# bibendovsky/oalsfxpp

Measured on AMD Instinct MI355X. Metric: Msamples/sec EAX reverb, 256-frame buffers, batch=4096; % HBM roofline, higher is better.
Workload: dtype f32

## Files before the change

### oalsfxpp_amd/csrc/hip/wave_effects_body.hpp

```cpp
#ifndef OALSFX_HIP_WAVE_EFFECTS_BODY_HPP
#define OALSFX_HIP_WAVE_EFFECTS_BODY_HPP

#include "common.hpp"

namespace oalsfx_hip {

namespace wfx {

constexpr int kRow = 68;
constexpr int kLdsRows = 20;
constexpr int kCoefBase = kLdsRows * kRow;
constexpr int kLdsFloats = kCoefBase + 32;

typedef __attribute__((address_space(1))) float GlobalFloat;
typedef const __attribute__((address_space(4))) oalsfx_slot_params ConstSlotParams;

struct Coef { float b0, b1, b2, a1, a2; };
template <class B> __device__ __forceinline__ Coef coef(const B& b) { return Coef{b.b0, b.b1, b.b2, b.a1, b.a2}; }

__device__ __forceinline__ void wave_sync()
{
    __builtin_amdgcn_fence(__ATOMIC_RELEASE, "wavefront");
    __builtin_amdgcn_wave_barrier();
    __builtin_amdgcn_fence(__ATOMIC_ACQUIRE, "wavefront");
}

template <int N>
__device__ __forceinline__ void chain_biquad_whole(float* row, float a1, float a2)
{
    static_assert(N % 32 == 0, "two blocks of sixteen per round");
    float y1 = row[3], y2 = row[2];
    auto step4 = [&](float4& v) {
        v.x = (v.x - (a1 * y1)) - (a2 * y2);
        v.y = (v.y - (a1 * v.x)) - (a2 * y1);
        v.z = (v.z - (a1 * v.y)) - (a2 * v.x);
        v.w = (v.w - (a1 * v.z)) - (a2 * v.y);
        y2 = v.z;
        y1 = v.w;
    };
    float4* r4 = reinterpret_cast<float4*>(row + 4);
    float4 a0 = r4[0], a1v = r4[1], a2v = r4[2], a3 = r4[3];
    float4 b0 = r4[4], b1 = r4[5], b2 = r4[6], b3 = r4[7];
    step4(a0); step4(a1v); step4(a2v); step4(a3);
    r4[0] = a0; r4[1] = a1v; r4[2] = a2v; r4[3] = a3;
    a0 = r4[8]; a1v = r4[9]; a2v = r4[10]; a3 = r4[11];
    step4(b0); step4(b1); step4(b2); step4(b3);
#pragma unroll 1
    for (int q = 8; q < N / 4; q += 8) {
        r4[q - 4] = b0; r4[q - 3] = b1; r4[q - 2] = b2; r4[q - 1] = b3;
        b0 = r4[q + 4]; b1 = r4[q + 5]; b2 = r4[q + 6]; b3 = r4[q + 7];
        step4(a0); step4(a1v); step4(a2v); step4(a3);
        r4[q + 0] = a0; r4[q + 1] = a1v; r4[q + 2] = a2v; r4[q + 3] = a3;
        a0 = r4[q + 8]; a1v = r4[q + 9]; a2v = r4[q + 10]; a3 = r4[q + 11];
        step4(b0); step4(b1); step4(b2); step4(b3);
    }
    r4[N / 4 - 4] = b0; r4[N / 4 - 3] = b1; r4[N / 4 - 2] = b2; r4[N / 4 - 1] = b3;
}

__device__ __forceinline__ void chain_biquad(float* row, int lo, int hi, float a1, float a2)
{
    float y1 = row[4 + lo - 1], y2 = row[4 + lo - 2];
    int i = lo;
    auto step4 = [&](float4& v) {
        v.x = (v.x - (a1 * y1)) - (a2 * y2);
        v.y = (v.y - (a1 * v.x)) - (a2 * y1);
        v.z = (v.z - (a1 * v.y)) - (a2 * v.x);
        v.w = (v.w - (a1 * v.z)) - (a2 * v.y);
        y2 = v.z;
        y1 = v.w;
    };
    if ((lo & 3) == 0 && lo + 16 <= hi) {
        float4* r4 = reinterpret_cast<float4*>(row + 4);
        float4 c0 = r4[(lo >> 2) + 0], c1 = r4[(lo >> 2) + 1], c2 = r4[(lo >> 2) + 2], c3 = r4[(lo >> 2) + 3];
        for (; i + 32 <= hi; i += 32) {
            const int q = i >> 2;
            float4 n0 = r4[q + 4], n1 = r4[q + 5], n2 = r4[q + 6], n3 = r4[q + 7];
            step4(c0); step4(c1); step4(c2); step4(c3);
            r4[q + 0] = c0; r4[q + 1] = c1; r4[q + 2] = c2; r4[q + 3] = c3;
            if (i + 48 <= hi) { c0 = r4[q + 8]; c1 = r4[q + 9]; c2 = r4[q + 10]; c3 = r4[q + 11]; }
            step4(n0); step4(n1); step4(n2); step4(n3);
            r4[q + 4] = n0; r4[q + 5] = n1; r4[q + 6] = n2; r4[q + 7] = n3;
        }
        if (i + 16 <= hi) {
            const int q = i >> 2;
            step4(c0); step4(c1); step4(c2); step4(c3);
            r4[q + 0] = c0; r4[q + 1] = c1; r4[q + 2] = c2; r4[q + 3] = c3;
            i += 16;
        }
    }
    for (; i < hi; ++i) {
        const float y = (row[4 + i] - (a1 * y1)) - (a2 * y2);
        row[4 + i] = y;
        y2 = y1;
        y1 = y;
    }
}

__device__ __forceinline__ void chain_first_order(float* row, int n, float c)
{
    float prev = row[3];
    int i = 0;
    if (n >= 16) {
        float4* r4 = reinterpret_cast<float4*>(row + 4);
        float4 c0 = r4[0], c1 = r4[1], c2 = r4[2], c3 = r4[3];
        auto step4 = [&](float4& v) {
            v.x = v.x + (c * prev);
            v.y = v.y + (c * v.x);
            v.z = v.z + (c * v.y);
            v.w = v.w + (c * v.z);
            prev = v.w;
        };
        for (; i + 32 <= n; i += 32) {
            const int q = i >> 2;
            float4 n0 = r4[q + 4], n1 = r4[q + 5], n2 = r4[q + 6], n3 = r4[q + 7];
            step4(c0); step4(c1); step4(c2); step4(c3);
            r4[q + 0] = c0; r4[q + 1] = c1; r4[q + 2] = c2; r4[q + 3] = c3;
            if (i + 48 <= n) { c0 = r4[q + 8]; c1 = r4[q + 9]; c2 = r4[q + 10]; c3 = r4[q + 11]; }
            step4(n0); step4(n1); step4(n2); step4(n3);
            r4[q + 4] = n0; r4[q + 5] = n1; r4[q + 6] = n2; r4[q + 7] = n3;
        }
        if (i + 16 <= n) {
            const int q = i >> 2;
            step4(c0); step4(c1); step4(c2); step4(c3);
            r4[q + 0] = c0; r4[q + 1] = c1; r4[q + 2] = c2; r4[q + 3] = c3;
            i += 16;
        }
    }
    for (; i < n; ++i) {
        prev = row[4 + i] + (c * prev);
        row[4 + i] = prev;
    }
}

__device__ __forceinline__ void advance_row(float* row, int n)
{
    if (n >= 2) {
        const float a = row[4 + n - 2], b = row[4 + n - 1];
        row[2] = a; row[3] = b;
    } else if (n == 1) {
        row[2] = row[3]; row[3] = row[4];
    }
}

__device__ __forceinline__ void load_hist(float* xrow, float* yrow, const oalsfx_hist_t& h)
{
    xrow[2] = h.x[1]; xrow[3] = h.x[0];
    yrow[2] = h.y[1]; yrow[3] = h.y[0];
}

__device__ __forceinline__ void store_hist(const float* xrow, const float* yrow, oalsfx_hist_t& h)
{
    h.x[1] = xrow[2]; h.x[0] = xrow[3];
    h.y[1] = yrow[2]; h.y[0] = yrow[3];
}

template <class T, class = void> struct LagOf { static constexpr int value = 0; };
template <class T> struct LagOf<T, decltype(void(T::kLag))> { static constexpr int value = T::kLag; };

struct Inst {
    ConstSlotParams* sp;
    oalsfx_slot_state* ss;
    GlobalFloat* ring;
    float* lds;
    int lane;
    int channels;
    bool coop;
    int wib;
    int duty;
    mutable int phase;
    float* group_lds;
    int group_stride;
};

__device__ __forceinline__ void lds_barrier()
{
    asm volatile("s_waitcnt lgkmcnt(0)\n\ts_barrier" ::: "memory");
}

template <class F>
__device__ __forceinline__ void chain_phase(const Inst& I, int lines, F&& f)
{
    if (!I.coop) {
        wave_sync();
        if (I.lane < lines) f(I.lds, I.lane);
        wave_sync();
    } else {
        const int duty = (I.duty + I.phase++) & 3;
        lds_barrier();
        if (I.wib == duty && I.lane < 4 * lines) f(I.group_lds + (I.lane / lines) * I.group_stride, I.lane % lines);
        lds_barrier();
    }
}

__device__ __forceinline__ float std_max(float a, float b) { return (a < b) ? b : a; }
__device__ __forceinline__ float std_min(float a, float b) { return (b < a) ? b : a; }

template <int CH, class G>
__device__ __forceinline__ void pan(float out[CH], int channels, const G& gains, float v)
{
#pragma unroll
    for (int c = 0; c < CH; ++c) {
        const float g = gains[c];
        if (c < channels && audible(g)) out[c] += g * v;
    }
}

struct NullW {
    __device__ void init(const Inst&) {}
    template <int CH> __device__ void tile(const Inst&, const float*, float*, int) {}
    __device__ void finish(const Inst&) {}
};

struct DedicatedW {
    __device__ void init(const Inst&) {}
    template <int CH> __device__ void tile(const Inst& I, const float* wet, float* out, int)
    {
        const auto& p = I.sp->u.dedicated;
#pragma unroll
        for (int c = 0; c < CH; ++c) {
            const float g = p.gains[c];
            if (c < I.channels && audible(g)) out[c] += wet[0] * g;
        }
    }
    __device__ void finish(const Inst&) {}
};

struct ModDelayW {
    int offset;
    float v_next[2];
    bool have_next, may_ask;
    __device__ void init(const Inst& I)
    {
        const auto& p = I.sp->u.moddelay;
        offset = I.ss->u.moddelay.offset;
        may_ask = p.delay - static_cast<int>(fabsf(p.depth)) - 1 >= 128;
        have_next = false;
        v_next[0] = v_next[1] = 0.0F;
    }
    template <class P> __device__ static int lfo_delay(const P& p, int phase)
    {
        if (p.waveform == 1) return static_cast<int>((1.0F - fabsf(2.0F - (p.lfo_scale * phase))) * p.depth) + p.delay;
        return static_cast<int>(glibc_sinf(p.lfo_scale * phase) * p.depth) + p.delay;
    }
    template <int CH> __device__ void tile(const Inst& I, const float* wet, float* out, int L)
    {
        const auto& p = I.sp->u.moddelay;
        const int lane = I.lane;
        const unsigned mask = static_cast<unsigned>(p.ring_len - 1);
        const int o = offset + lane;
        const float in = wet[0];
        const float fb = p.feedback;
        float t[2];
        int d[2];
        bool inside[2];
        float v[2];
        if (have_next) {
#pragma unroll
            for (int k = 0; k < 2; ++k) {
                d[k] = 128;
                inside[k] = false;
                v[k] = lane < L ? v_next[k] : in;
            }
        } else {
#pragma unroll
            for (int k = 0; k < 2; ++k) {
                const GlobalFloat* buf = I.ring + (k ? p.ring_len : 0);
                const int phase = (k ? o + p.lfo_disp : o) % p.lfo_range;
                d[k] = lfo_delay(p, phase);
                inside[k] = d[k] > 0 && lane - d[k] >= 0;
                v[k] = in;
                if (lane < L && d[k] != 0 && !inside[k]) v[k] = buf[static_cast<unsigned>(o - d[k]) & mask];
            }
        }
        have_next = false;
        if (may_ask && L == 64) {
            int dn[2];
#pragma unroll
            for (int k = 0; k < 2; ++k) dn[k] = lfo_delay(p, (k ? o + 64 + p.lfo_disp : o + 64) % p.lfo_range);
            have_next = __ballot(dn[0] < 128 || dn[1] < 128) == 0ULL;
            if (have_next) {
#pragma unroll
                for (int k = 0; k < 2; ++k) v_next[k] = (I.ring + (k ? p.ring_len : 0))[static_cast<unsigned>(o + 64 - dn[k]) & mask];
            }
        }
        float val[2] = {0.0F, 0.0F};
        t[0] = t[1] = 0.0F;
        int s[2] = {0, 0};
#pragma unroll
        for (int k = 0; k < 2; ++k) {
            const unsigned long long in_tile = __ballot(inside[k] && lane < L);
            if (in_tile == 0ULL) continue;
            const int d0 = __builtin_amdgcn_readlane(d[k], static_cast<int>(__builtin_ctzll(in_tile)));
            if (d0 > 16 || __ballot(lane >= d0 && lane < L && d[k] != d0) != 0ULL) continue;
            const int chain = lane % d0, step = lane / d0;
            float* row = I.lds + chain * kRow;
            const float head_t = v[k] * fb;
            if (lane < L) row[3 + step] = step == 0 ? in + head_t : in;
            wave_sync();
            if (lane < d0 && lane < L) chain_first_order(I.lds + lane * kRow, (L - lane + d0 - 1) / d0 - 1, fb);
            wave_sync();
            if (lane < L) {
                val[k] = row[3 + step];
                t[k] = step == 0 ? head_t : row[2 + step] * fb;
            }
            wave_sync();
            s[k] = L;
        }
        while (s[0] < L || s[1] < L) {
            int e[2];
            float handed[2];
#pragma unroll
            for (int k = 0; k < 2; ++k) {
                const bool blocked = lane >= s[k] && lane < L && inside[k] && lane - d[k] >= s[k];
                const unsigned long long nb = __ballot(blocked);
                e[k] = nb ? static_cast<int>(__builtin_ctzll(nb)) : L;
                handed[k] = __shfl(val[k], inside[k] ? lane - d[k] : lane);
            }
#pragma unroll
            for (int k = 0; k < 2; ++k) {
                if (lane >= s[k] && lane < L && lane < e[k]) {
                    if (inside[k]) v[k] = handed[k];
                    t[k] = v[k] * fb;
                    val[k] = in + t[k];
                }
                s[k] = max(s[k], e[k]);
            }
        }
#pragma unroll
        for (int k = 0; k < 2; ++k) {
            GlobalFloat* buf = I.ring + (k ? p.ring_len : 0);
            if (lane < L) buf[static_cast<unsigned>(o) & mask] = val[k];
        }
#pragma unroll
        for (int k = 0; k < 2; ++k) pan<CH>(out, I.channels, p.gains[k], t[k]);
        offset += L;
        wave_sync();
    }
    __device__ void finish(const Inst& I)
    {
        if (I.lane == 0) I.ss->u.moddelay.offset = offset;
    }
};

struct CompressorW {
    __device__ void init(const Inst& I)
    {
        if (I.lane == 0) {
            I.lds[3] = I.ss->u.compressor.gain_control;
            I.lds[0] = I.sp->u.compressor.attack_rate;
            I.lds[1] = I.sp->u.compressor.release_rate;
        }
        wave_sync();
    }
    template <int CH> __device__ void tile(const Inst& I, const float* wet, float* out, int L)
    {
        const auto& p = I.sp->u.compressor;
        float* row = I.lds;
        float amplitude = 1.0F;
        if (p.enabled) {
            amplitude = fabsf(wet[0]);
            amplitude = std_max(amplitude + fabsf(wet[1]), std_max(amplitude + fabsf(wet[2]), amplitude + fabsf(wet[3])));
        }
        row[4 + I.lane] = amplitude;
        chain_phase(I, 1, [L](float* row, int) {
            float gc = row[3];
            const float attack = row[0], release = row[1];
            auto follow = [&](float a) {
                if (a > gc) gc = std_min(gc + attack, a);
                else if (a < gc) gc = std_max(gc - release, a);
                return gc;
            };
            int i = 0;
            if (L >= 4) {
                float4 a = *reinterpret_cast<const float4*>(row + 4);
                for (; i + 4 <= L; i += 4) {
                    float4 an = a;
                    if (i + 8 <= L) an = *reinterpret_cast<const float4*>(row + 8 + i);
                    float4 g;
                    g.x = follow(a.x); g.y = follow(a.y); g.z = follow(a.z); g.w = follow(a.w);
                    *reinterpret_cast<float4*>(row + 4 + i) = g;
                    a = an;
                }
            }
            for (; i < L; ++i) row[4 + i] = follow(row[4 + i]);
            row[3] = gc;
        });
        const float output = 1.0F / std_min(2.0F, std_max(0.5F, row[4 + I.lane]));
        wave_sync();
#pragma unroll
        for (int j = 0; j < 4; ++j) pan<CH>(out, I.channels, p.gains[j], wet[j] * output);
    }
    __device__ void finish(const Inst& I)
    {
        if (I.lane == 0) I.ss->u.compressor.gain_control = I.lds[3];
    }
};

struct EqualizerW {
    static constexpr int kBlock = 16;
    __device__ void init(const Inst& I)
    {
        const oalsfx_equalizer_state& s = I.ss->u.equalizer;
        if (I.lane < 16) {
            const int b = I.lane >> 2, ch = I.lane & 3;
            load_hist(I.lds + (b * 4 + ch) * kRow, I.lds + ((b + 1) * 4 + ch) * kRow, s.hist[b][ch]);
        }
        if (I.lane < 4) {
            const auto& band = I.sp->u.equalizer.band[I.lane];
            float* cf = I.lds + kCoefBase + 8 * I.lane;
            cf[0] = band.b0; cf[1] = band.b1; cf[2] = band.b2; cf[3] = band.a1; cf[4] = band.a2;
        }
        wave_sync();
    }
    __device__ static void filter_block(const float* xrow, float* yrow, int n0, int n1, const float* cf)
    {
        const float b0 = cf[0], b1 = cf[1], b2 = cf[2], a1 = cf[3], a2 = cf[4];
        float x1 = xrow[4 + n0 - 1], x2 = xrow[4 + n0 - 2], y1 = yrow[4 + n0 - 1], y2 = yrow[4 + n0 - 2];
        auto step = [&](float x0) {
            const float u = ((b0 * x0) + (b1 * x1)) + (b2 * x2);
            const float y = (u - (a1 * y1)) - (a2 * y2);
            x2 = x1; x1 = x0; y2 = y1; y1 = y;
            return y;
        };
        if (n1 - n0 == kBlock) {
            const float4* x4 = reinterpret_cast<const float4*>(xrow + 4 + n0);
            float4* y4 = reinterpret_cast<float4*>(yrow + 4 + n0);
            float4 v[4] = {x4[0], x4[1], x4[2], x4[3]};
#pragma unroll
            for (int k = 0; k < 4; ++k) {
                v[k].x = step(v[k].x); v[k].y = step(v[k].y); v[k].z = step(v[k].z); v[k].w = step(v[k].w);
            }
#pragma unroll
            for (int k = 0; k < 4; ++k) y4[k] = v[k];
        } else {
            for (int n = n0; n < n1; ++n) yrow[4 + n] = step(xrow[4 + n]);
        }
    }
    template <int CH> __device__ void tile(const Inst& I, const float* wet, float* out, int L)
    {
        const auto& p = I.sp->u.equalizer;
        const int lane = I.lane;
#pragma unroll
        for (int ch = 0; ch < 4; ++ch) I.lds[ch * kRow + 4 + lane] = wet[ch];
        chain_phase(I, 16, [L](float* lds, int line) {
            const int b = line >> 2, ch = line & 3;
            const float* xrow = lds + (b * 4 + ch) * kRow;
            float* yrow = lds + ((b + 1) * 4 + ch) * kRow;
            const float* cf = lds + kCoefBase + 8 * b;
            const int blocks = (L + kBlock - 1) / kBlock;
            for (int r = 0; r < blocks + 3; ++r) {
                const int k = r - b;
                if (k >= 0 && k < blocks) filter_block(xrow, yrow, k * kBlock, min(L, (k + 1) * kBlock), cf);
                wave_sync();
            }
        });
#pragma unroll
        for (int ch = 0; ch < 4; ++ch) pan<CH>(out, I.channels, p.gains[ch], I.lds[(16 + ch) * kRow + 4 + lane]);
        wave_sync();
        if (lane < 20) advance_row(I.lds + lane * kRow, L);
        wave_sync();
    }
    __device__ void finish(const Inst& I)
    {
        oalsfx_equalizer_state& s = I.ss->u.equalizer;
        if (I.lane < 16) {
            const int b = I.lane >> 2, ch = I.lane & 3;
            store_hist(I.lds + (b * 4 + ch) * kRow, I.lds + ((b + 1) * 4 + ch) * kRow, s.hist[b][ch]);
        }
    }
};

struct RingModW {
    int index;
    __device__ void init(const Inst& I)
    {
        const oalsfx_ringmod_state& s = I.ss->u.ringmod;
        index = s.index;
        if (I.lane < 4) {
            load_hist(I.lds + I.lane * kRow, I.lds + (4 + I.lane) * kRow, s.hist[I.lane]);
            float* yrow = I.lds + (4 + I.lane) * kRow;
            yrow[0] = I.sp->u.ringmod.filter.a1;
            yrow[1] = I.sp->u.ringmod.filter.a2;
        }
        wave_sync();
    }
    __device__ static float carrier(int waveform, int idx)
    {
        constexpr int frac_bits = 24;
        constexpr int frac_one = 1 << frac_bits;
        if (waveform == 0) return glibc_sinf(idx * (6.28318530717958647692F / frac_one) - 3.14159265358979323846F) * 0.5F + 0.5F;
        if (waveform == 1) return static_cast<float>(idx) / frac_one;
        return static_cast<float>((idx >> (frac_bits - 1)) & 1);
    }
    template <int CH> __device__ void tile(const Inst& I, const float* wet, float* out, int L)
    {
        const auto& p = I.sp->u.ringmod;
        const int lane = I.lane;
        const Coef c = coef(p.filter);
#pragma unroll
        for (int ch = 0; ch < 4; ++ch) I.lds[ch * kRow + 4 + lane] = wet[ch];
        wave_sync();
#pragma unroll
        for (int ch = 0; ch < 4; ++ch) {
            const float* x = I.lds + ch * kRow + 4 + lane;
            I.lds[(4 + ch) * kRow + 4 + lane] = ((c.b0 * x[0]) + (c.b1 * x[-1])) + (c.b2 * x[-2]);
        }
        chain_phase(I, 4, [L](float* lds, int line) {
            float* row = lds + (4 + line) * kRow;
            chain_biquad(row, 0, L, row[0], row[1]);
        });
        const unsigned frac_mask = (1u << 24) - 1u;
        const int idx = static_cast<int>((static_cast<unsigned>(index) + static_cast<unsigned>(lane + 1) * static_cast<unsigned>(p.step)) & frac_mask);
        const float m = carrier(p.waveform, idx);
#pragma unroll
        for (int ch = 0; ch < 4; ++ch) pan<CH>(out, I.channels, p.gains[ch], I.lds[(4 + ch) * kRow + 4 + lane] * m);
        index = static_cast<int>((static_cast<unsigned>(index) + static_cast<unsigned>(L) * static_cast<unsigned>(p.step)) & frac_mask);
        wave_sync();
        if (lane < 8) advance_row(I.lds + lane * kRow, L);
        wave_sync();
    }
    __device__ void finish(const Inst& I)
    {
        oalsfx_ringmod_state& s = I.ss->u.ringmod;
        if (I.lane < 4) store_hist(I.lds + I.lane * kRow, I.lds + (4 + I.lane) * kRow, s.hist[I.lane]);
        if (I.lane == 0) s.index = index;
    }
};

struct EchoW {
    int offset;
    float n_t1, n_t2;
    bool have_next;
    int block;
    __device__ void init(const Inst& I)
    {
        const auto& p = I.sp->u.echo;
        offset = I.ss->u.echo.offset;
        n_t1 = n_t2 = 0.0F;
        have_next = false;
        block = max(1, min(64, p.tap2 > 0 ? p.tap2 : 64));
        if (I.lane == 0) {
            load_hist(I.lds, I.lds + kRow, I.ss->u.echo.filter);
            float* yrow = I.lds + kRow;
            yrow[0] = p.filter.a1; yrow[1] = p.filter.a2;
            if (I.coop) reinterpret_cast<int*>(I.lds + kCoefBase)[0] = block;
        }
        wave_sync();
        if (I.coop) {
            lds_barrier();
#pragma unroll
            for (int k = 0; k < 4; ++k) block = min(block, reinterpret_cast<const int*>(I.group_lds + k * I.group_stride + kCoefBase)[0]);
        }
    }
    template <int CH> __device__ void tile(const Inst& I, const float* wet, float* out, int L)
    {
        const auto& p = I.sp->u.echo;
        const int lane = I.lane;
        const unsigned mask = static_cast<unsigned>(p.ring_len - 1);
        const Coef c = coef(p.filter);
        const int o = offset + lane;
        float* xrow = I.lds;
        float* yrow = I.lds + kRow;
        float* wrow = I.lds + 2 * kRow;
        const bool in1 = p.tap1 > 0 && lane - p.tap1 >= 0, in2 = p.tap2 > 0 && lane - p.tap2 >= 0;
        float t1 = 0.0F, t2 = 0.0F;
        if (have_next) {
            t1 = n_t1; t2 = n_t2;
        } else if (lane < L) {
            if (!in1) t1 = I.ring[static_cast<unsigned>(o - p.tap1) & mask];
            if (!in2) t2 = I.ring[static_cast<unsigned>(o - p.tap2) & mask];
        }
        have_next = L == 64 && p.tap1 >= 128 && p.tap2 >= 128;
        if (have_next) {
            n_t1 = I.ring[static_cast<unsigned>(o + 64 - p.tap1) & mask];
            n_t2 = I.ring[static_cast<unsigned>(o + 64 - p.tap2) & mask];
        }
        for (int s = 0; s < L; s += block) {
            const int e = min(L, s + block);
            const bool mine = lane >= s && lane < e;
            if (mine) {
                if (in2) t2 = wrow[4 + lane - p.tap2];
                xrow[4 + lane] = t2 + wet[0];
            }
            wave_sync();
            if (mine) {
                const float* x = xrow + 4 + lane;
                yrow[4 + lane] = ((x[0] * c.b0) + (x[-1] * c.b1)) + (x[-2] * c.b2);
            }
            chain_phase(I, 1, [s, e](float* lds, int) {
                float* row = lds + kRow;
                chain_biquad(row, s, e, row[0], row[1]);
            });
            if (mine) wrow[4 + lane] = yrow[4 + lane] * p.feed_gain;
            wave_sync();
        }
        if (lane < L) I.ring[static_cast<unsigned>(o) & mask] = wrow[4 + lane];
        if (in1 && lane < L) t1 = wrow[4 + lane - p.tap1];
#pragma unroll
        for (int ch = 0; ch < CH; ++ch) {
            if (ch >= I.channels) continue;
            const float g0 = p.gains[0][ch];
            if (audible(g0)) out[ch] += t1 * g0;
            const float g1 = p.gains[1][ch];
            if (audible(g1)) out[ch] += t2 * g1;
        }
        offset += L;
        wave_sync();
        if (lane < 2) advance_row(I.lds + lane * kRow, L);
        wave_sync();
    }
    __device__ void finish(const Inst& I)
    {
        if (I.lane == 0) {
            store_hist(I.lds, I.lds + kRow, I.ss->u.echo.filter);
            I.ss->u.echo.offset = offset;
        }
    }
};

struct DistortionW {
    static constexpr int kArr = 4 + 4 * 64;
    float x_hist0, x_hist1;
    __device__ void init(const Inst& I)
    {
        const oalsfx_distortion_state& s = I.ss->u.distortion;
        x_hist0 = s.low_pass.x[0];
        x_hist1 = s.low_pass.x[1];
        if (I.lane == 0) {
            float* lp = I.lds; float* sh = I.lds + kArr; float* bp = I.lds + 2 * kArr;
            lp[2] = s.low_pass.y[1]; lp[3] = s.low_pass.y[0];
            sh[2] = s.band_pass.x[1]; sh[3] = s.band_pass.x[0];
            bp[2] = s.band_pass.y[1]; bp[3] = s.band_pass.y[0];
            lp[0] = I.sp->u.distortion.low_pass.a1; lp[1] = I.sp->u.distortion.low_pass.a2;
            bp[0] = I.sp->u.distortion.band_pass.a1; bp[1] = I.sp->u.distortion.band_pass.a2;
        }
        wave_sync();
    }
    static constexpr int kLag = 1;
    template <int CH> __device__ void tile(const Inst& I, const float* wet, float* out, int L, int Lp)
    {
        const auto& p = I.sp->u.distortion;
        const int lane = I.lane;
        float* lp = I.lds; float* sh = I.lds + kArr; float* bp = I.lds + 2 * kArr;
        const int n = 4 * L, np = 4 * Lp;
        if (L > 0) {
            const Coef c = coef(p.low_pass);
            const float X = wet[0] * 4.0F;
            const float z = 0.0F;
            const float p1 = lane == 0 ? x_hist0 : z;
            const float p2 = lane == 0 ? x_hist1 : z;
            float4 u;
            u.x = ((c.b0 * X) + (c.b1 * p1)) + (c.b2 * p2);
            u.y = ((c.b0 * z) + (c.b1 * X)) + (c.b2 * p1);
            u.z = ((c.b0 * z) + (c.b1 * z)) + (c.b2 * X);
            u.w = ((c.b0 * z) + (c.b1 * z)) + (c.b2 * z);
            *reinterpret_cast<float4*>(lp + 4 + 4 * lane) = u;
        }
        chain_phase(I, 2, [n, np](float* lds, int line) {
            float* row = lds + (line ? 2 * kArr : 0);
            const int cnt = line ? np : n;
            if (cnt == 256) chain_biquad_whole<256>(row, row[0], row[1]);
            else chain_biquad(row, 0, cnt, row[0], row[1]);
        });
        if (Lp > 0) {
            const float kept = bp[4 + 4 * lane];
#pragma unroll
            for (int c = 0; c < CH; ++c) {
                const float g = p.gains[c] * p.attenuation;
                if (c < I.channels && audible(g)) out[c] += g * kept;
            }
        }
        wave_sync();
        if (lane == 0) advance_row(bp, np);
        if (L > 0) {
            const float h2 = sh[2], h1 = sh[3];
            const float4 y = *reinterpret_cast<const float4*>(lp + 4 + 4 * lane);
            const float fc = p.edge_coeff;
            auto shape = [fc](float smp) {
                smp = (1.0F + fc) * smp / (1.0F + (fc * fabsf(smp)));
                smp = (1.0F + fc) * smp / (1.0F + (fc * fabsf(smp))) * -1.0F;
                smp = (1.0F + fc) * smp / (1.0F + (fc * fabsf(smp)));
                return smp;
            };
            const float x0 = shape(y.x), x1 = shape(y.y), x2 = shape(y.z), x3 = shape(y.w);
            float p1 = __shfl_up(x3, 1), p2 = __shfl_up(x2, 1);
            if (lane == 0) { p1 = h1; p2 = h2; }
            const Coef c = coef(p.band_pass);
            float4 u;
            u.x = ((c.b0 * x0) + (c.b1 * p1)) + (c.b2 * p2);
            u.y = ((c.b0 * x1) + (c.b1 * x0)) + (c.b2 * p1);
            u.z = ((c.b0 * x2) + (c.b1 * x1)) + (c.b2 * x0);
            u.w = ((c.b0 * x3) + (c.b1 * x2)) + (c.b2 * x1);
            *reinterpret_cast<float4*>(bp + 4 + 4 * lane) = u;
            if (lane == L - 1) { sh[2] = x2; sh[3] = x3; }
            if (lane == 0) advance_row(lp, n);
            x_hist0 = 0.0F; x_hist1 = 0.0F;
            wave_sync();
        }
    }
    __device__ void finish(const Inst& I)
    {
        if (I.lane == 0) {
            oalsfx_distortion_state& s = I.ss->u.distortion;
            const float* lp = I.lds; const float* sh = I.lds + kArr; const float* bp = I.lds + 2 * kArr;
            s.low_pass.x[0] = x_hist0; s.low_pass.x[1] = x_hist1;
            s.low_pass.y[1] = lp[2]; s.low_pass.y[0] = lp[3];
            s.band_pass.x[1] = sh[2]; s.band_pass.x[0] = sh[3];
            s.band_pass.y[1] = bp[2]; s.band_pass.y[0] = bp[3];
        }
    }
};

static_assert(3 * DistortionW::kArr <= kLdsFloats, "distortion arrays must fit the per-wave LDS");

struct Group {
    bool coop;
    int wib, duty;
    float* lds;
    int stride;
};

template <int CH, class Fx>
__device__ __forceinline__ void wave_instance(const KernelCtx& ctx, int slot, int inst, int flags, float* lds, int lane, const Group& group)
{
    const int channels = (CH == 8) ? ctx.channels : CH;
    const int frames = ctx.frames;
    const size_t sidx = static_cast<size_t>(inst) * ctx.slots + slot;
    typedef const __attribute__((address_space(4))) oalsfx_source_params ConstSourceParams;
    ConstSourceParams& SRC = *(ConstSourceParams*)(uintptr_t)(ctx.source + inst);
    const bool first = (flags & kFirst) != 0;
    const bool last = (flags & kLast) != 0;
    const bool filtered = (flags & kFiltered) != 0 && instance_has_send_filter(ctx, inst);
    const float* src = ctx.raw_src + static_cast<size_t>(inst) * ctx.io_stride;
    const float* wsrc = src;
    if (filtered) {
        src = ctx.src + static_cast<size_t>(inst) * ctx.src_stride;
        wsrc = ctx.wet_src + static_cast<size_t>(inst) * ctx.src_stride;
    }
    float* dst = ctx.dst + static_cast<size_t>(inst) * ctx.io_stride;
    float* mixbuf = ctx.mixbuf ? ctx.mixbuf + static_cast<size_t>(inst) * channels * OALSFX_MAX_CHUNK : nullptr;
    const bool send_on = SRC.aux[slot].out_channels != 0;

    Inst I;
    I.sp = (ConstSlotParams*)(uintptr_t)(ctx.params + sidx);
    I.ss = ctx.state + sidx;
    I.ring = (GlobalFloat*)(uintptr_t)ctx.rings[sidx];
    I.lds = lds;
    I.lane = lane;
    I.channels = channels;
    I.coop = group.coop;
    I.wib = group.wib;
    I.duty = group.duty;
    I.phase = 0;
    I.group_lds = group.lds;
    I.group_stride = group.stride;

    int ts_i = 0;
    auto stamp = [&]() {
        if (ctx.timeline && (inst & 63) == 0 && (inst >> 6) < 64 && lane == 0 && ts_i < 24)
            ctx.timeline[64 * 4 * 96 + (inst >> 6) * 96 + (slot & 3) * 24 + ts_i++] = clock64();
    };
    stamp();
    Fx fx;

    float n_in[CH], n_win[CH], n_mix[CH];
    auto request = [&](int base) {
        const int p = base + lane;
        const bool a = p < frames;
#pragma unroll
        for (int c = 0; c < CH; ++c) { n_in[c] = 0.0F; n_mix[c] = 0.0F; }
        if (a) {
            if (CH == 2) {
                const float2 v = *reinterpret_cast<const float2*>(src + static_cast<size_t>(p) * 2);
                n_in[0] = v.x; n_in[CH - 1] = v.y;
            } else {
#pragma unroll
                for (int c = 0; c < CH; ++c)
                    if (c < channels) n_in[c] = src[static_cast<size_t>(p) * channels + c];
            }
        }
#pragma unroll
        for (int c = 0; c < CH; ++c) n_win[c] = n_in[c];
        if (filtered && a) {
#pragma unroll
            for (int c = 0; c < CH; ++c)
                if (c < channels) n_win[c] = wsrc[static_cast<size_t>(p) * channels + c];
        }
        if (!first && a) {
#pragma unroll
            for (int c = 0; c < CH; ++c)
                if (c < channels) n_mix[c] = mixbuf[c * OALSFX_MAX_CHUNK + p];
        }
    };
    auto store_tile = [&](const float* o, int p, bool a) {
        if (!a) return;
        if (last && ctx.turn_set != 0u && CH <= 2) {
            if (CH == 2) {
                const unsigned long long both = static_cast<unsigned long long>(__float_as_uint(o[0])) | (static_cast<unsigned long long>(__float_as_uint(o[CH - 1])) << 32);
                __hip_atomic_store(reinterpret_cast<unsigned long long*>(dst + static_cast<size_t>(p) * 2), both, __ATOMIC_RELAXED, __HIP_MEMORY_SCOPE_AGENT);
            } else {
                __hip_atomic_store(reinterpret_cast<unsigned*>(dst + p), __float_as_uint(o[0]), __ATOMIC_RELAXED, __HIP_MEMORY_SCOPE_AGENT);
            }
        } else if (last) {
            if (CH == 2) {
                *reinterpret_cast<float2*>(dst + static_cast<size_t>(p) * 2) = make_float2(o[0], o[CH - 1]);
            } else {
#pragma unroll
                for (int c = 0; c < CH; ++c)
                    if (c < channels) dst[static_cast<size_t>(p) * channels + c] = o[c];
            }
        } else {
#pragma unroll
            for (int c = 0; c < CH; ++c)
                if (c < channels) mixbuf[c * OALSFX_MAX_CHUNK + p] = o[c];
        }
    };
    constexpr int kLag = LagOf<Fx>::value;
    float held[CH];
    int held_pos = 0, held_L = 0;
#pragma unroll
    for (int c = 0; c < CH; ++c) held[c] = 0.0F;
    request(0);
    fx.init(I);
    stamp();
    for (int base = 0; base < frames + (kLag ? 64 : 0); base += 64) {
        const int L = base < frames ? min(64, frames - base) : 0;
        const bool act = lane < L;
        const int pos = base + lane;
        float in[CH], win[CH], out[CH];
#pragma unroll
        for (int c = 0; c < CH; ++c) { in[c] = n_in[c]; win[c] = n_win[c]; out[c] = 0.0F; }
        float mix[CH];
#pragma unroll
        for (int c = 0; c < CH; ++c) mix[c] = n_mix[c];
        if (base + 64 < frames) request(base + 64);
        __builtin_amdgcn_sched_barrier(0);
        float wet[4] = {0.0F, 0.0F, 0.0F, 0.0F};
#pragma unroll
        for (int c = 0; c < CH; ++c) {
            if (c >= channels) continue;
            if (first) {
#pragma unroll
                for (int o = 0; o < CH; ++o) {
                    const float g = SRC.direct.gains[c][o];
                    if (o < channels && audible(g)) out[o] += in[c] * g;
                }
            }
            if (send_on) {
#pragma unroll
                for (int k = 0; k < 4; ++k) {
                    const float g = SRC.aux[slot].gains[c][k];
                    if (audible(g)) wet[k] += win[c] * g;
                }
            }
        }
        if (!first) {
#pragma unroll
            for (int c = 0; c < CH; ++c) out[c] = mix[c];
        }
        stamp();
        if constexpr (kLag != 0) {
            fx.template tile<CH>(I, wet, held, L, held_L);
            stamp();
            store_tile(held, held_pos, lane < held_L);
#pragma unroll
            for (int c = 0; c < CH; ++c) held[c] = out[c];
            held_pos = pos;
            held_L = L;
        } else {
            fx.template tile<CH>(I, wet, out, L);
            stamp();
            store_tile(out, pos, act);
        }
    }

    fx.finish(I);
    if (lane == 0) I.ss->seen_seq = I.sp->update_seq;
    if (first && !filtered && lane < channels) send_history_follow(ctx, inst, lane, channels, frames, src);
}


template <int CH>
__device__ __forceinline__ void wave_slots(const KernelCtx& ctx, int slot, int slot_count, int inst, int flags, float* lds, int lane, const Group& group)
{
    for (int sl = slot; sl < slot + slot_count; ++sl) {
        const int f = (flags & kFiltered) | ((flags & kFirst) && sl == slot ? kFirst : 0) | ((flags & kLast) && sl == slot + slot_count - 1 ? kLast : 0);
        const int type = __builtin_amdgcn_readfirstlane(ctx.params[static_cast<size_t>(inst) * ctx.slots + sl].type);
        KernelCtx c = ctx;
        c.wet_src = ctx.wet_src + static_cast<size_t>(sl - slot) * ctx.wet_plane;
        switch (type) {
        case OALSFX_NULL:
            if (f & (kFirst | kLast)) wave_instance<CH, NullW>(c, sl, inst, f, lds, lane, group);
            break;
        case OALSFX_CHORUS:
        case OALSFX_FLANGER: wave_instance<CH, ModDelayW>(c, sl, inst, f, lds, lane, group); break;
        case OALSFX_COMPRESSOR: wave_instance<CH, CompressorW>(c, sl, inst, f, lds, lane, group); break;
        case OALSFX_DEDICATED_DIALOG:
        case OALSFX_DEDICATED_LFE: wave_instance<CH, DedicatedW>(c, sl, inst, f, lds, lane, group); break;
        case OALSFX_DISTORTION: wave_instance<CH, DistortionW>(c, sl, inst, f, lds, lane, group); break;
        case OALSFX_ECHO: wave_instance<CH, EchoW>(c, sl, inst, f, lds, lane, group); break;
        case OALSFX_EQUALIZER: wave_instance<CH, EqualizerW>(c, sl, inst, f, lds, lane, group); break;
        case OALSFX_RING_MODULATOR: wave_instance<CH, RingModW>(c, sl, inst, f, lds, lane, group); break;
        default: break;
        }
        wave_sync();
    }
}

template <int CH, bool CHN = false>
__device__ __forceinline__ void wave_block(const KernelCtx& ctx, int slot, int slot_count, const int* __restrict__ list, int count,
                                           const WaveSegments& seg, int flags, int block, float* lds_group, int lds_stride)
{
    const int lane = threadIdx.x & 63;
    const int wib = __builtin_amdgcn_readfirstlane(threadIdx.x >> 6);
    if (CHN && ctx.turn_started != nullptr && threadIdx.x == 0) __hip_atomic_fetch_add(ctx.turn_started, 1u, __ATOMIC_RELAXED, __HIP_MEMORY_SCOPE_AGENT);
    Group group{false, wib, block & 3, lds_group, lds_stride};
    int w = block * 4 + wib;
    if (seg.n > 0) {
        int k = 0, first_block = 0;
        for (; k + 1 < seg.n; ++k) {
            const int b = (seg.count[k] + 3) >> 2;
            if (block < first_block + b) break;
            first_block += b;
        }
        const int local = (block - first_block) * 4 + wib;
        group.coop = ((seg.coop_mask >> k) & 1u) != 0;
        if (local >= seg.count[k]) return;
        w = seg.offset[k] + local;
    } else {
        if (CHN && !((flags >> 8) & 8)) w = cu_major_position(block, (count + 3) >> 2) * 4 + wib;
        if (w >= count) return;
    }
    const int inst = __builtin_amdgcn_readfirstlane(list[w]);
    unsigned cu_before = 0;
    const size_t word = static_cast<size_t>(inst) * ctx.slots + ctx.turn_slot;
    if (CHN && ((flags >> 8) & 4) && ctx.turn != nullptr && ctx.turn_wait != 0u) {
        unsigned junk = 0;
        for (int sl = slot; sl < slot + slot_count; ++sl) {
            const unsigned* st = reinterpret_cast<const unsigned*>(ctx.state + static_cast<size_t>(inst) * ctx.slots + sl);
#pragma unroll
            for (int k = 0; k < static_cast<int>(sizeof(SlotStateLines) / 256); ++k) {
                unsigned a;
                asm volatile("global_load_dword %0, %1, off\n\ts_waitcnt vmcnt(0)" : "=v"(a) : "v"(st + 64 * k + lane) : "memory");
                junk ^= a;
            }
        }
        if (ctx.mixbuf != nullptr) {
            const unsigned* mb = reinterpret_cast<const unsigned*>(ctx.mixbuf + static_cast<size_t>(inst) * ctx.channels * OALSFX_MAX_CHUNK);
            for (int c = 0; c < ctx.channels; ++c) {
                unsigned a;
                asm volatile("global_load_dword %0, %1, off\n\ts_waitcnt vmcnt(0)" : "=v"(a) : "v"(mb + c * OALSFX_MAX_CHUNK + 32 * lane) : "memory");
                junk ^= a;
            }
        }
        if (junk == 0x7E57AB1Eu && ctx.timeline) ctx.timeline[0] = junk;
    }
    const bool mine = !CHN || turn_take(ctx, word, lane, flags >> 8, cu_before);
    if (CHN && group.coop) { if (__syncthreads_or(mine ? 0 : 1)) return; }
    else if (!mine) return;
    wave_slots<CH>(ctx, slot, slot_count, inst, flags, lds_group + wib * lds_stride, lane, group);
    if (CHN) turn_hand_on(ctx, word, lane, cu_before);
}

}

}

#endif
```

Measured before the change: 28750.

## Software-pipeline front-end mixing and pin loads to hide global memory latency

Moves the per-tile input mixing (direct gains and send gains) into a front_end lambda that runs for the next tile inside or right after the effect tile. Empty inline-asm 'land' constraints force prefetched loads to complete at chosen points, so their latency overlaps effect work. For CH<=2 the direct and send gains are hoisted into scalar registers once. This raises register pressure and makes ordering depend on compiler barriers, which could cost occupancy.

```diff
diff --git a/oalsfxpp_amd/csrc/hip/wave_effects_body.hpp b/oalsfxpp_amd/csrc/hip/wave_effects_body.hpp
--- a/oalsfxpp_amd/csrc/hip/wave_effects_body.hpp
+++ b/oalsfxpp_amd/csrc/hip/wave_effects_body.hpp
@@ -157,6 +157,12 @@
 template <class T, class = void> struct LagOf { static constexpr int value = 0; };
 template <class T> struct LagOf<T, decltype(void(T::kLag))> { static constexpr int value = T::kLag; };
 
+template <class T, class = void> struct LandsInputs { static constexpr bool value = false; };
+template <class T> struct LandsInputs<T, decltype(void(T::kLandsInputs))> { static constexpr bool value = T::kLandsInputs; };
+
+template <class T> __device__ __forceinline__ void land_vector(T& v) { static_assert(sizeof(T) == 4, "one register"); asm volatile("" : "+v"(v)); }
+__device__ __forceinline__ void pin_scalar(float& s) { asm volatile("" : "+s"(s)); }
+
 struct Inst {
     ConstSlotParams* sp;
     oalsfx_slot_state* ss;
@@ -233,6 +239,7 @@
     {
         const auto& p = I.sp->u.moddelay;
         offset = I.ss->u.moddelay.offset;
+        land_vector(offset);
         may_ask = p.delay - static_cast<int>(fabsf(p.depth)) - 1 >= 128;
         have_next = false;
         v_next[0] = v_next[1] = 0.0F;
@@ -242,7 +249,8 @@
         if (p.waveform == 1) return static_cast<int>((1.0F - fabsf(2.0F - (p.lfo_scale * phase))) * p.depth) + p.delay;
         return static_cast<int>(glibc_sinf(p.lfo_scale * phase) * p.depth) + p.delay;
     }
-    template <int CH> __device__ void tile(const Inst& I, const float* wet, float* out, int L)
+    static constexpr bool kLandsInputs = true;
+    template <int CH, class Land> __device__ void tile(const Inst& I, const float* wet, float* out, int L, Land&& land)
     {
         const auto& p = I.sp->u.moddelay;
         const int lane = I.lane;
@@ -264,13 +272,18 @@
         } else {
 #pragma unroll
             for (int k = 0; k < 2; ++k) {
-                const GlobalFloat* buf = I.ring + (k ? p.ring_len : 0);
                 const int phase = (k ? o + p.lfo_disp : o) % p.lfo_range;
                 d[k] = lfo_delay(p, phase);
                 inside[k] = d[k] > 0 && lane - d[k] >= 0;
                 v[k] = in;
+            }
+#pragma unroll
+            for (int k = 0; k < 2; ++k) {
+                const GlobalFloat* buf = I.ring + (k ? p.ring_len : 0);
                 if (lane < L && d[k] != 0 && !inside[k]) v[k] = buf[static_cast<unsigned>(o - d[k]) & mask];
             }
+            land_vector(v[0]);
+            land_vector(v[1]);
         }
         have_next = false;
         if (may_ask && L == 64) {
@@ -326,6 +339,9 @@
                 s[k] = max(s[k], e[k]);
             }
         }
+        land_vector(v_next[0]);
+        land_vector(v_next[1]);
+        land();
 #pragma unroll
         for (int k = 0; k < 2; ++k) {
             GlobalFloat* buf = I.ring + (k ? p.ring_len : 0);
@@ -476,6 +492,7 @@
     {
         const oalsfx_ringmod_state& s = I.ss->u.ringmod;
         index = s.index;
+        land_vector(index);
         if (I.lane < 4) {
             load_hist(I.lds + I.lane * kRow, I.lds + (4 + I.lane) * kRow, s.hist[I.lane]);
             float* yrow = I.lds + (4 + I.lane) * kRow;
@@ -536,6 +553,7 @@
     {
         const auto& p = I.sp->u.echo;
         offset = I.ss->u.echo.offset;
+        land_vector(offset);
         n_t1 = n_t2 = 0.0F;
         have_next = false;
         block = max(1, min(64, p.tap2 > 0 ? p.tap2 : 64));
@@ -552,7 +570,8 @@
             for (int k = 0; k < 4; ++k) block = min(block, reinterpret_cast<const int*>(I.group_lds + k * I.group_stride + kCoefBase)[0]);
         }
     }
-    template <int CH> __device__ void tile(const Inst& I, const float* wet, float* out, int L)
+    static constexpr bool kLandsInputs = true;
+    template <int CH, class Land> __device__ void tile(const Inst& I, const float* wet, float* out, int L, Land&& land)
     {
         const auto& p = I.sp->u.echo;
         const int lane = I.lane;
@@ -566,9 +585,13 @@
         float t1 = 0.0F, t2 = 0.0F;
         if (have_next) {
             t1 = n_t1; t2 = n_t2;
-        } else if (lane < L) {
-            if (!in1) t1 = I.ring[static_cast<unsigned>(o - p.tap1) & mask];
-            if (!in2) t2 = I.ring[static_cast<unsigned>(o - p.tap2) & mask];
+        } else {
+            if (lane < L) {
+                if (!in1) t1 = I.ring[static_cast<unsigned>(o - p.tap1) & mask];
+                if (!in2) t2 = I.ring[static_cast<unsigned>(o - p.tap2) & mask];
+            }
+            land_vector(t1);
+            land_vector(t2);
         }
         have_next = L == 64 && p.tap1 >= 128 && p.tap2 >= 128;
         if (have_next) {
@@ -594,6 +617,9 @@
             if (mine) wrow[4 + lane] = yrow[4 + lane] * p.feed_gain;
             wave_sync();
         }
+        land_vector(n_t1);
+        land_vector(n_t2);
+        land();
         if (lane < L) I.ring[static_cast<unsigned>(o) & mask] = wrow[4 + lane];
         if (in1 && lane < L) t1 = wrow[4 + lane - p.tap1];
 #pragma unroll
@@ -626,6 +652,8 @@
         const oalsfx_distortion_state& s = I.ss->u.distortion;
         x_hist0 = s.low_pass.x[0];
         x_hist1 = s.low_pass.x[1];
+        land_vector(x_hist0);
+        land_vector(x_hist1);
         if (I.lane == 0) {
             float* lp = I.lds; float* sh = I.lds + kArr; float* bp = I.lds + 2 * kArr;
             lp[2] = s.low_pass.y[1]; lp[3] = s.low_pass.y[0];
@@ -763,12 +791,24 @@
     stamp();
     Fx fx;
 
+    constexpr bool kHoldGains = CH <= 2;
+    float g_direct[kHoldGains ? CH * CH : 1], g_send[kHoldGains ? CH * 4 : 1];
+    if constexpr (kHoldGains) {
+#pragma unroll
+        for (int c = 0; c < CH; ++c) {
+#pragma unroll
+            for (int o = 0; o < CH; ++o) { g_direct[c * CH + o] = SRC.direct.gains[c][o]; pin_scalar(g_direct[c * CH + o]); }
+#pragma unroll
+            for (int k = 0; k < 4; ++k) { g_send[c * 4 + k] = SRC.aux[slot].gains[c][k]; pin_scalar(g_send[c * 4 + k]); }
+        }
+    }
+
     float n_in[CH], n_win[CH], n_mix[CH];
     auto request = [&](int base) {
         const int p = base + lane;
         const bool a = p < frames;
 #pragma unroll
-        for (int c = 0; c < CH; ++c) { n_in[c] = 0.0F; n_mix[c] = 0.0F; }
+        for (int c = 0; c < CH; ++c) { n_in[c] = 0.0F; n_win[c] = 0.0F; n_mix[c] = 0.0F; }
         if (a) {
             if (CH == 2) {
                 const float2 v = *reinterpret_cast<const float2*>(src + static_cast<size_t>(p) * 2);
@@ -779,8 +819,6 @@
                     if (c < channels) n_in[c] = src[static_cast<size_t>(p) * channels + c];
             }
         }
-#pragma unroll
-        for (int c = 0; c < CH; ++c) n_win[c] = n_in[c];
         if (filtered && a) {
 #pragma unroll
             for (int c = 0; c < CH; ++c)
@@ -820,56 +858,77 @@
     int held_pos = 0, held_L = 0;
 #pragma unroll
     for (int c = 0; c < CH; ++c) held[c] = 0.0F;
+    float f_out[CH], f_wet[4];
+    auto front_end = [&]() {
+#pragma unroll
+        for (int c = 0; c < CH; ++c) { land_vector(n_in[c]); land_vector(n_win[c]); land_vector(n_mix[c]); }
+#pragma unroll
+        for (int c = 0; c < CH; ++c) f_out[c] = 0.0F;
+#pragma unroll
+        for (int k = 0; k < 4; ++k) f_wet[k] = 0.0F;
+#pragma unroll
+        for (int c = 0; c < CH; ++c) {
+            if (c >= channels) continue;
+            const float in = n_in[c], win = filtered ? n_win[c] : n_in[c];
+            if (first) {
+#pragma unroll
+                for (int o = 0; o < CH; ++o) {
+                    float g;
+                    if constexpr (kHoldGains) g = g_direct[c * CH + o];
+                    else g = SRC.direct.gains[c][o];
+                    if (o < channels && audible(g)) f_out[o] += in * g;
+                }
+            }
+            if (send_on) {
+#pragma unroll
+                for (int k = 0; k < 4; ++k) {
+                    float g;
+                    if constexpr (kHoldGains) g = g_send[c * 4 + k];
+                    else g = SRC.aux[slot].gains[c][k];
+                    if (audible(g)) f_wet[k] += win * g;
+                }
+            }
+        }
+        if (!first) {
+#pragma unroll
+            for (int c = 0; c < CH; ++c) f_out[c] = n_mix[c];
+        }
+        __builtin_amdgcn_sched_barrier(0);
+    };
     request(0);
     fx.init(I);
     stamp();
+    front_end();
     for (int base = 0; base < frames + (kLag ? 64 : 0); base += 64) {
         const int L = base < frames ? min(64, frames - base) : 0;
         const bool act = lane < L;
         const int pos = base + lane;
-        float in[CH], win[CH], out[CH];
-#pragma unroll
-        for (int c = 0; c < CH; ++c) { in[c] = n_in[c]; win[c] = n_win[c]; out[c] = 0.0F; }
-        float mix[CH];
-#pragma unroll
-        for (int c = 0; c < CH; ++c) mix[c] = n_mix[c];
+        float out[CH], wet[4];
+#pragma unroll
+        for (int c = 0; c < CH; ++c) out[c] = f_out[c];
+#pragma unroll
+        for (int k = 0; k < 4; ++k) wet[k] = f_wet[k];
         if (base + 64 < frames) request(base + 64);
         __builtin_amdgcn_sched_barrier(0);
-        float wet[4] = {0.0F, 0.0F, 0.0F, 0.0F};
-#pragma unroll
-        for (int c = 0; c < CH; ++c) {
-            if (c >= channels) continue;
-            if (first) {
-#pragma unroll
-                for (int o = 0; o < CH; ++o) {
-                    const float g = SRC.direct.gains[c][o];
-                    if (o < channels && audible(g)) out[o] += in[c] * g;
-                }
-            }
-            if (send_on) {
-#pragma unroll
-                for (int k = 0; k < 4; ++k) {
-                    const float g = SRC.aux[slot].gains[c][k];
-                    if (audible(g)) wet[k] += win[c] * g;
-                }
-            }
-        }
-        if (!first) {
-#pragma unroll
-            for (int c = 0; c < CH; ++c) out[c] = mix[c];
-        }
+        auto land = [&]() { front_end(); };
         stamp();
         if constexpr (kLag != 0) {
             fx.template tile<CH>(I, wet, held, L, held_L);
             stamp();
+            land();
             store_tile(held, held_pos, lane < held_L);
 #pragma unroll
             for (int c = 0; c < CH; ++c) held[c] = out[c];
             held_pos = pos;
             held_L = L;
+        } else if constexpr (LandsInputs<Fx>::value) {
+            fx.template tile<CH>(I, wet, out, L, land);
+            stamp();
+            store_tile(out, pos, act);
         } else {
             fx.template tile<CH>(I, wet, out, L);
             stamp();
+            land();
             store_tile(out, pos, act);
         }
     }
```

Result: no change. 28660 (median of 2 runs) (-0.3%).
